# Dhia-naouali/dinov3-jax

Hardware: NVIDIA H100
Metric: global_crops_per_sec (higher is better)
Workload: dtype bf16

## Files before the change

dinov3-jax_b200/csrc/gemm_tc.cu:

```cuda
#include <cstdlib>
#include <cstring>
#include "ptx.cuh"
#include "d3_internal.h"

namespace d3 {

constexpr int BM = 128;
constexpr int BK = 64;
constexpr int GEMM_THREADS = 384;

constexpr int EPI_RUNTIME = -1;
constexpr int EPI_FLAGS = EP_BIAS | EP_GELU | EP_STORE_PRE | EP_MUL_DGELU | EP_GAMMA | EP_RESID | EP_OUT_F32 | EP_ACCUM |
                          EP_SLABS | EP_GELU_ERF;

template <int EF>
constexpr bool kStaged = EF != EPI_RUNTIME && (EF & (EP_SLABS | EP_ACCUM)) == 0;

template <int EF>
__device__ __forceinline__ bool epi_has(const GemmEpilogue& ep, int f) {
  return EF == EPI_RUNTIME ? (ep.flags & f) != 0 : (EF & f) != 0;
}

__device__ __forceinline__ float gelu_grad_epi(float u) {
  const float u2 = __fmul_rn(u, u);
  const float t = tanh_approx(__fmul_rn(u, fmaf(0.0356774081363001f, u2, 0.7978845608028654f)));
  const float dz = fmaf(0.1070322244089003f, u2, 0.7978845608028654f);
  return fmaf(__fmul_rn(__fmul_rn(0.5f, u), fmaf(-t, t, 1.0f)), dz, __fmul_rn(0.5f, __fadd_rn(1.0f, t)));
}

__device__ __forceinline__ float gelu_erf_epi(float u) {
  return __fmul_rn(__fmul_rn(0.5f, u), __fadd_rn(1.0f, erff(__fmul_rn(u, 0.70710678118654752f))));
}

template <int EF>
__device__ __forceinline__ float epi_value(const GemmEpilogue& ep, float acc, float bias, float u, float gamma,
                                           float resid, float old, float& pre) {
  float v = __fmul_rn(acc, ep.alpha);
  if (epi_has<EF>(ep, EP_BIAS)) v = __fadd_rn(v, bias);
  pre = v;
  if (epi_has<EF>(ep, EP_GELU)) v = gelu_tanh_fast(v);
  if (epi_has<EF>(ep, EP_GELU_ERF)) v = gelu_erf_epi(v);
  if (epi_has<EF>(ep, EP_MUL_DGELU)) v = __fmul_rn(v, gelu_grad_epi(u));
  if (epi_has<EF>(ep, EP_GAMMA)) v = __fmul_rn(v, gamma);
  if (epi_has<EF>(ep, EP_RESID)) v = __fadd_rn(v, resid);
  if (epi_has<EF>(ep, EP_ACCUM)) v = __fadd_rn(v, old);
  return v;
}

__device__ __forceinline__ float2 ld_pair(const float* p, bool vec, bool two) {
  if (vec) return *reinterpret_cast<const float2*>(p);
  return make_float2(p[0], two ? p[1] : 0.f);
}
__device__ __forceinline__ float2 ld_pair(const __nv_bfloat16* p, bool vec, bool two) {
  if (vec) return unpack_bf16(*reinterpret_cast<const uint32_t*>(p));
  return make_float2(__bfloat162float(p[0]), two ? __bfloat162float(p[1]) : 0.f);
}
__device__ __forceinline__ void st_pair(float* p, float a, float b, bool vec, bool two) {
  if (vec) {
    *reinterpret_cast<float2*>(p) = make_float2(a, b);
  } else {
    p[0] = a;
    if (two) p[1] = b;
  }
}
__device__ __forceinline__ void st_pair(__nv_bfloat16* p, float a, float b, bool vec, bool two) {
  if (vec) {
    *reinterpret_cast<uint32_t*>(p) = pack_bf16(a, b);
  } else {
    p[0] = __float2bfloat16(a);
    if (two) p[1] = __float2bfloat16(b);
  }
}

template <int BN>
__device__ __forceinline__ void epilogue_tile_runtime(const GemmEpilogue& ep, float (&acc)[2][BN / 2], int m0, int n0,
                                                      int M, int N, size_t slab_row0, int r_in, int c_in) {
  float* const out_f = reinterpret_cast<float*>(ep.out);
  __nv_bfloat16* const out_h = reinterpret_cast<__nv_bfloat16*>(ep.out);
  const bool aligned = (ep.flags & EP_SLOW) == 0;
#pragma unroll
  for (int mh = 0; mh < 2; ++mh)
#pragma unroll
    for (int h = 0; h < 2; ++h) {
      const size_t row = (size_t)(m0 + mh * 64 + r_in + 8 * h);
      if (row >= (size_t)M) continue;
      const size_t orow = slab_row0 + row;
#pragma unroll
      for (int i = 0; i < BN / 8; ++i) {
        const int n = n0 + 8 * i + c_in;
        if (n >= N) break;
        const bool two = n + 1 < N, vec = aligned && two;
        float2 b{}, u{}, g{}, x{}, o{};
        if (epi_has<EPI_RUNTIME>(ep, EP_BIAS)) b = ld_pair(ep.bias + n, vec, two);
        if (epi_has<EPI_RUNTIME>(ep, EP_MUL_DGELU)) u = ld_pair(ep.aux_in + row * ep.ld_aux + n, vec, two);
        if (epi_has<EPI_RUNTIME>(ep, EP_GAMMA)) g = ld_pair(ep.gamma + n, vec, two);
        if (epi_has<EPI_RUNTIME>(ep, EP_RESID)) x = ld_pair(ep.resid + row * ep.ld_resid + n, vec, two);
        if (epi_has<EPI_RUNTIME>(ep, EP_ACCUM)) o = ld_pair(out_f + orow * ep.ld_out + n, vec, two);
        float p0, p1;
        const float v0 = epi_value<EPI_RUNTIME>(ep, acc[mh][4 * i + 2 * h], b.x, u.x, g.x, x.x, o.x, p0);
        const float v1 = epi_value<EPI_RUNTIME>(ep, acc[mh][4 * i + 2 * h + 1], b.y, u.y, g.y, x.y, o.y, p1);
        if (epi_has<EPI_RUNTIME>(ep, EP_SCATTER)) {
          const unsigned long long g_idx = (unsigned long long)ep.sc_off + orow * ep.ld_out + n;
          const unsigned long long shard = (unsigned long long)ep.sc_shard;
          const unsigned r = (unsigned)(g_idx / shard);
          float* const dst = ep.sc_peer[r] + (g_idx - r * shard);
          if (!two) atomicAdd(dst, v0);
          else atomicAdd(reinterpret_cast<float2*>(dst), make_float2(v0, v1));
          continue;
        }
        if (epi_has<EPI_RUNTIME>(ep, EP_STORE_PRE)) st_pair(ep.aux_out + row * ep.ld_aux + n, p0, p1, vec, two);
        if (epi_has<EPI_RUNTIME>(ep, EP_OUT_F32)) st_pair(out_f + orow * ep.ld_out + n, v0, v1, vec, two);
        else st_pair(out_h + orow * ep.ld_out + n, v0, v1, vec, two);
      }
    }
}

constexpr int STG_BOX = 64 * 128;
constexpr int STG_BYTES = 3 * STG_BOX;
__device__ __forceinline__ uint32_t sw128(int r, int byte) {
  return r * 128 + ((((byte >> 4) ^ r) & 7) << 4) + (byte & 15);
}

template <int MH, int BN, int EF>
__device__ __forceinline__ void epilogue_tile(const GemmEpilogue& ep, const CUtensorMap* tm_out,
                                              const CUtensorMap* tm_pre, float (&acc)[MH][BN / 2], const float* s_bias,
                                              const float* s_gamma, uint8_t* stg, int& seq, int bar, int t, int m0,
                                              int n0, int M, int N, size_t slab_row0, int r_in, int c_in) {
  constexpr bool STAGED = kStaged<EF>;
  constexpr bool F32 = (EF & EP_OUT_F32) != 0;
  constexpr int OUT_BOXES = F32 ? 2 : 1;
  constexpr int CHUNK = (OUT_BOXES + ((EF & EP_STORE_PRE) ? 1 : 0)) * STG_BOX;
  constexpr int NBUF = STG_BYTES / CHUNK;
  static_assert(NBUF >= 1, "a chunk must fit the staging area");
  float* const out_f = reinterpret_cast<float*>(ep.out);
  __nv_bfloat16* const out_h = reinterpret_cast<__nv_bfloat16*>(ep.out);
#pragma unroll
  for (int mh = 0; mh < MH; ++mh)
#pragma unroll
    for (int cb = 0; cb < BN / 64; ++cb) {
      const int row0 = m0 + mh * 64, col0 = n0 + cb * 64;
      if (row0 >= M || col0 >= N) continue;
      float2 xr[2][8], xo[2][8];
      uint32_t xu[2][8];
#pragma unroll
      for (int h = 0; h < 2; ++h) {
        const size_t row = (size_t)row0 + r_in + 8 * h;
#pragma unroll
        for (int i = 0; i < 8; ++i) {
          const int n = col0 + 8 * i + c_in;
          if (row < (size_t)M && n < N) {
            if (epi_has<EF>(ep, EP_RESID))
              xr[h][i] = *reinterpret_cast<const float2*>(ep.resid + row * ep.ld_resid + n);
            if (epi_has<EF>(ep, EP_MUL_DGELU))
              xu[h][i] = *reinterpret_cast<const uint32_t*>(ep.aux_in + row * ep.ld_aux + n);
            if (epi_has<EF>(ep, EP_ACCUM))
              xo[h][i] = *reinterpret_cast<const float2*>(out_f + (slab_row0 + row) * ep.ld_out + n);
          }
        }
      }
      uint8_t* const buf = stg + (seq % NBUF) * CHUNK;
      if constexpr (STAGED) {
        if (t == 0) tma_store_wait_read<NBUF - 1>();
        named_bar_sync(bar, 128);
      }
#pragma unroll
      for (int h = 0; h < 2; ++h) {
        const int r = r_in + 8 * h;
        const size_t row = (size_t)row0 + r;
#pragma unroll
        for (int i = 0; i < 8; ++i) {
          const int cl = cb * 64 + 8 * i + c_in;
          const int n = n0 + cl;
          const float2 b = epi_has<EF>(ep, EP_BIAS) ? *reinterpret_cast<const float2*>(s_bias + cl) : float2{};
          const float2 g = epi_has<EF>(ep, EP_GAMMA) ? *reinterpret_cast<const float2*>(s_gamma + cl) : float2{};
          const float2 u = epi_has<EF>(ep, EP_MUL_DGELU) ? unpack_bf16(xu[h][i]) : float2{};
          float p0, p1;
          const float v0 = epi_value<EF>(ep, acc[mh][4 * (cl >> 3) + 2 * h], b.x, u.x, g.x, xr[h][i].x, xo[h][i].x, p0);
          const float v1 = epi_value<EF>(ep, acc[mh][4 * (cl >> 3) + 2 * h + 1], b.y, u.y, g.y, xr[h][i].y, xo[h][i].y,
                                         p1);
          if constexpr (STAGED) {
            if (epi_has<EF>(ep, EP_STORE_PRE))
              *reinterpret_cast<uint32_t*>(buf + OUT_BOXES * STG_BOX + sw128(r, 16 * i + 2 * c_in)) = pack_bf16(p0, p1);
            if constexpr (F32) {
              *reinterpret_cast<float2*>(buf + (i >> 2) * STG_BOX + sw128(r, 32 * (i & 3) + 4 * c_in)) =
                  make_float2(v0, v1);
            } else {
              *reinterpret_cast<uint32_t*>(buf + sw128(r, 16 * i + 2 * c_in)) = pack_bf16(v0, v1);
            }
          } else if (row < (size_t)M && n < N) {
            if (epi_has<EF>(ep, EP_STORE_PRE)) st_pair(ep.aux_out + row * ep.ld_aux + n, p0, p1, true, true);
            if constexpr (F32) st_pair(out_f + (slab_row0 + row) * ep.ld_out + n, v0, v1, true, true);
            else st_pair(out_h + (slab_row0 + row) * ep.ld_out + n, v0, v1, true, true);
          }
        }
      }
      if constexpr (STAGED) {
        fence_proxy_async_smem();
        named_bar_sync(bar, 128);
        if (t == 0) {
          tma_store_2d(tm_out, buf, col0, row0);
          if (F32 && col0 + 32 < N) tma_store_2d(tm_out, buf + STG_BOX, col0 + 32, row0);
          if constexpr ((EF & EP_STORE_PRE) != 0) tma_store_2d(tm_pre, buf + OUT_BOXES * STG_BOX, col0, row0);
          tma_store_commit();
        }
        ++seq;
      }
    }
}

template <int BN, bool STAGED>
struct Cfg {
  static constexpr bool WIDE = BN == 256;
  static constexpr int STAGES = (BN == 256 ? 4 : BN == 128 ? 6 : 8) - (STAGED ? 1 : 0);
  static constexpr int A_BYTES = BM * BK * 2;
  static constexpr int B_BYTES = BN * BK * 2;
  static constexpr int STAGE_BYTES = A_BYTES + B_BYTES;
  static constexpr int BAR_BYTES = 256;
  static constexpr int VEC_BYTES = (WIDE ? 1 : 2) * 2 * BN * 4;
  static constexpr int VEC_END = STAGES * STAGE_BYTES + BAR_BYTES + VEC_BYTES;
  static constexpr int STG_OFF = (VEC_END + 1023) / 1024 * 1024;
  static constexpr int SMEM_BYTES = (STAGED ? STG_OFF + 2 * STG_BYTES : VEC_END) + 1024;
  static_assert(SMEM_BYTES <= 227 * 1024, "over the opt-in shared-memory limit");
};

struct WorkRange { int m0, n0, kb0, kb1, sp; };
template <int BN>
__device__ __forceinline__ WorkRange work_item(int w, int rank, int num_n, int num_tiles, int num_k, int splits) {
  const int tile = w % num_tiles, sp = w / num_tiles;
  const int per = (num_k + splits - 1) / splits;
  WorkRange r;
  if constexpr (BN == 256) {
    r.n0 = (tile % num_n) * BN;
    r.m0 = (2 * (tile / num_n) + rank) * BM;
  } else {
    r.n0 = (2 * (tile % num_n) + rank) * BN;
    r.m0 = (tile / num_n) * BM;
  }
  r.kb0 = sp * per;
  r.kb1 = min(num_k, r.kb0 + per);
  r.sp = sp;
  return r;
}

template <int MH, int BN, int A_MN, int B_MN>
__device__ __forceinline__ void mma_kblock(float (&acc)[MH][BN / 2], uint32_t sa, uint32_t sb, bool first) {
  const uint64_t bd = B_MN ? gmma_desc_sw128(sb, 8192, 1024) : gmma_desc_sw128(sb, 16, 1024);
  constexpr uint64_t a_adv = A_MN ? (2048 >> 4) : (32 >> 4);
  constexpr uint64_t b_adv = B_MN ? (2048 >> 4) : (32 >> 4);
#pragma unroll
  for (int k = 0; k < BK / 16; ++k) {
    const uint32_t sc = (first && k == 0) ? 0u : 1u;
#pragma unroll
    for (int mh = 0; mh < MH; ++mh) {
      const uint64_t ad = A_MN ? gmma_desc_sw128(sa + mh * 8192, 8192, 1024) : gmma_desc_sw128(sa + mh * 8192, 16, 1024);
      if constexpr (BN == 256) wgmma_m64n256k16_ss<A_MN, B_MN>(acc[mh], ad + k * a_adv, bd + k * b_adv, sc);
      else if constexpr (BN == 128) wgmma_m64n128k16_ss<A_MN, B_MN>(acc[mh], ad + k * a_adv, bd + k * b_adv, sc);
      else wgmma_m64n64k16_ss<A_MN, B_MN>(acc[mh], ad + k * a_adv, bd + k * b_adv, sc);
    }
  }
}

template <int MH, int BN>
__device__ __forceinline__ void mma_khalf_e4m3(float (&acc)[MH][BN / 2], uint32_t sa, uint32_t sb, int h) {
  static_assert(BN == 64, "the e4m3 GEMM runs 128 x 64 tiles");
  const uint64_t bd = gmma_desc_sw128(sb, 16, 1024);
#pragma unroll
  for (int k = 0; k < 2; ++k) {
#pragma unroll
    for (int mh = 0; mh < MH; ++mh) {
      const uint64_t ad = gmma_desc_sw128(sa + mh * 8192, 16, 1024);
      wgmma_m64n64k32_e4m3(acc[mh], ad + (2 * h + k) * (32 >> 4), bd + (2 * h + k) * (32 >> 4), k == 0 ? 0u : 1u);
    }
  }
}

template <int MH, int BN>
__device__ __forceinline__ void add_acc(float (&acc)[MH][BN / 2], const float (&part)[MH][BN / 2]) {
#pragma unroll
  for (int mh = 0; mh < MH; ++mh)
#pragma unroll
    for (int i = 0; i < BN / 2; ++i) acc[mh][i] = __fadd_rn(acc[mh][i], part[mh][i]);
}

template <int BN, int A_MN, int B_MN, int EF, bool E4M3 = false>
__global__ void __launch_bounds__(GEMM_THREADS, 1)
gemm_kernel(const __grid_constant__ CUtensorMap tmA, const __grid_constant__ CUtensorMap tmB,
            const __grid_constant__ CUtensorMap tmO, const __grid_constant__ CUtensorMap tmP, const GemmEpilogue ep,
            int M, int N, int K, int splits, const float* scale_a, const float* scale_b) {
  static_assert(!E4M3 || (BN == 64 && !A_MN && !B_MN), "e4m3: 128 x 64 tiles, both operands K-major");
  constexpr int KB = E4M3 ? 128 : BK;
  constexpr bool staged = kStaged<EF>;
  using C = Cfg<BN, staged>;
  constexpr bool WIDE = C::WIDE;
  constexpr int MH = WIDE ? 1 : 2;
  static_assert(!WIDE || EF != EPI_RUNTIME, "run-time flags run on the 128-wide tile");
  static_assert(2 * C::STAGES * 8 <= C::BAR_BYTES, "mbarriers overflow their slot");
  extern __shared__ uint8_t smem_raw[];
  uint8_t* smem = reinterpret_cast<uint8_t*>((reinterpret_cast<uintptr_t>(smem_raw) + 1023) & ~uintptr_t(1023));
  uint64_t* full_bar = reinterpret_cast<uint64_t*>(smem + C::STAGES * C::STAGE_BYTES);
  uint64_t* empty_bar = full_bar + C::STAGES;
  float* vecs = reinterpret_cast<float*>(smem + C::STAGES * C::STAGE_BYTES + C::BAR_BYTES);

  const int wg = threadIdx.x >> 7;
  const int rank = blockIdx.x & 1;
  const int cluster = blockIdx.x >> 1, num_clusters = gridDim.x >> 1;
  if (threadIdx.x == 0) {
    tma_prefetch_desc(&tmA);
    tma_prefetch_desc(&tmB);
    if constexpr (staged) {
      tma_prefetch_desc(&tmO);
      if constexpr ((EF & EP_STORE_PRE) != 0) tma_prefetch_desc(&tmP);
    }
    for (int s = 0; s < C::STAGES; ++s) { mbar_init(&full_bar[s], 1); mbar_init(&empty_bar[s], WIDE ? 4 : 2); }
    fence_mbar_init();
  }
  cluster_sync();

  const int num_m = (M + BM - 1) / BM;
  const int num_n = WIDE ? (N + BN - 1) / BN : ((N + BN - 1) / BN + 1) / 2;
  const int num_k = (K + KB - 1) / KB;
  const int num_tiles = (WIDE ? (num_m + 1) / 2 : num_m) * num_n;
  const int num_work = num_tiles * splits;

  if (wg == 0) {
    setmaxnreg_dec<40>();
    if (threadIdx.x < 32 && elect_one()) {
      int stage = 0;
      uint32_t phase = 0;
      for (int w = cluster; w < num_work; w += num_clusters) {
        const WorkRange wr = work_item<BN>(w, rank, num_n, num_tiles, num_k, splits);
        for (int kb = wr.kb0; kb < wr.kb1; ++kb) {
          mbar_wait(&empty_bar[stage], phase ^ 1);
          uint8_t* sa = smem + stage * C::STAGE_BYTES;
          uint8_t* sb = sa + C::A_BYTES;
          mbar_expect_tx(&full_bar[stage], C::STAGE_BYTES);
          if constexpr (WIDE) {
#pragma unroll
            for (int i = 0; i < 2; ++i) {
              if (A_MN) tma_load_2d(&tmA, &full_bar[stage], sa + i * 8192, wr.m0 + i * 64, kb * KB);
              else tma_load_2d(&tmA, &full_bar[stage], sa + i * 8192, kb * KB, wr.m0 + i * 64);
            }
            if (B_MN) {
#pragma unroll
              for (int i = 2 * rank; i < 2 * rank + 2; ++i)
                tma_load_2d_multicast(&tmB, &full_bar[stage], sb + i * 8192, wr.n0 + i * 64, kb * KB, 0b11);
            } else {
              tma_load_2d_multicast(&tmB, &full_bar[stage], sb + rank * 16384, kb * KB, wr.n0 + rank * 128, 0b11);
            }
          } else {
            if (A_MN) {
              tma_load_2d_multicast(&tmA, &full_bar[stage], sa + rank * 8192, wr.m0 + rank * 64, kb * KB, 0b11);
            } else {
              tma_load_2d_multicast(&tmA, &full_bar[stage], sa + rank * 8192, kb * KB, wr.m0 + rank * 64, 0b11);
            }
            if (B_MN) {
#pragma unroll
              for (int i = 0; i < BN / 64; ++i) tma_load_2d(&tmB, &full_bar[stage], sb + i * 8192, wr.n0 + i * 64, kb * KB);
            } else {
              tma_load_2d(&tmB, &full_bar[stage], sb, kb * KB, wr.n0);
            }
          }
          if (++stage == C::STAGES) { stage = 0; phase ^= 1; }
        }
      }
    }
  } else {
    setmaxnreg_inc<232>();
    const int cw = wg - 1;
    const int t = threadIdx.x & 127;
    const int r_in = 16 * (t >> 5) + ((t & 31) >> 2);
    const int c_in = 2 * (t & 3);
    float* const s_bias = vecs + (WIDE ? 0 : cw * 2 * BN);
    float* const s_gamma = s_bias + BN;
    constexpr bool stage_vecs = EF != EPI_RUNTIME && (EF & (EP_BIAS | EP_GAMMA)) != 0;
    constexpr int VEC_THREADS = WIDE ? 256 : 128;
    const int vt = WIDE ? threadIdx.x - 128 : t;
    uint8_t* const stg = smem + C::STG_OFF + cw * STG_BYTES;
    const uint32_t peer_empty = mapa_shared(smem_u32(empty_bar), rank ^ 1);
    int stg_seq = 0;
    int stage = 0;
    uint32_t phase = 0;
    int j = 0;
    for (int w = cluster; w < num_work; w += num_clusters, ++j) {
      const WorkRange wr = work_item<BN>(w, rank, num_n, num_tiles, num_k, splits);
      const int nkb = wr.kb1 > wr.kb0 ? wr.kb1 - wr.kb0 : 0;
      if (!WIDE && (j & 1) != cw) {
        stage += nkb;
        phase ^= (stage / C::STAGES) & 1;
        stage %= C::STAGES;
        continue;
      }
      if constexpr (stage_vecs) {
        named_bar_sync(3 + cw * !WIDE, VEC_THREADS);
        if (vt < BN && wr.n0 + vt < N) {
          if constexpr ((EF & EP_BIAS) != 0) cp_async_4(s_bias + vt, ep.bias + wr.n0 + vt);
          if constexpr ((EF & EP_GAMMA) != 0) cp_async_4(s_gamma + vt, ep.gamma + wr.n0 + vt);
        }
      }
      if (!WIDE && j > 0) named_bar_sync(1 + cw, 256);
      float acc[MH][BN / 2];
#pragma unroll
      for (int mh = 0; mh < MH; ++mh)
#pragma unroll
        for (int i = 0; i < BN / 2; ++i) acc[mh][i] = 0.f;
      if constexpr (E4M3) {
        float part[MH][BN / 2];
        for (int kb = wr.kb0; kb < wr.kb1; ++kb) {
          mbar_wait(&full_bar[stage], phase);
          const uint32_t sa = smem_u32(smem + stage * C::STAGE_BYTES);
#pragma unroll
          for (int h = 0; h < 2; ++h) {
#pragma unroll
            for (int mh = 0; mh < MH; ++mh) fence_regs(part[mh]);
            wgmma_fence();
            mma_khalf_e4m3<MH, BN>(part, sa, sa + C::A_BYTES, h);
            wgmma_commit();
            wgmma_wait<0>();
#pragma unroll
            for (int mh = 0; mh < MH; ++mh) fence_regs(part[mh]);
            if (h == 1 && t == 0) { mbar_arrive(&empty_bar[stage]); mbar_arrive_cluster(peer_empty + 8 * stage); }
            add_acc<MH, BN>(acc, part);
          }
          if (++stage == C::STAGES) { stage = 0; phase ^= 1; }
        }
        if (!WIDE && w + num_clusters < num_work) named_bar_arrive(1 + (cw ^ 1), 256);
#pragma unroll
        for (int mh = 0; mh < MH; ++mh)
#pragma unroll
          for (int h = 0; h < 2; ++h) {
            const int row = wr.m0 + mh * 64 + r_in + 8 * h;
            const float s_row = row < M ? scale_a[row] : 0.f;
#pragma unroll
            for (int i = 0; i < BN / 8; ++i) {
              const int n = wr.n0 + 8 * i + c_in;
              const float s0 = n < N ? scale_b[n] : 0.f, s1 = n + 1 < N ? scale_b[n + 1] : 0.f;
              acc[mh][4 * i + 2 * h] = __fmul_rn(__fmul_rn(acc[mh][4 * i + 2 * h], s_row), s0);
              acc[mh][4 * i + 2 * h + 1] = __fmul_rn(__fmul_rn(acc[mh][4 * i + 2 * h + 1], s_row), s1);
            }
          }
      } else {
        int prev = -1;
        for (int kb = wr.kb0; kb < wr.kb1; ++kb) {
          mbar_wait(&full_bar[stage], phase);
          const uint32_t sa = smem_u32(smem + stage * C::STAGE_BYTES);
#pragma unroll
          for (int mh = 0; mh < MH; ++mh) fence_regs(acc[mh]);
          wgmma_fence();
          mma_kblock<MH, BN, A_MN, B_MN>(acc, sa + (WIDE ? cw * 8192 : 0), sa + C::A_BYTES, kb == wr.kb0);
          wgmma_commit();
#pragma unroll
          for (int mh = 0; mh < MH; ++mh) fence_regs(acc[mh]);
          if (prev >= 0) {
            wgmma_wait<1>();
            if (t == 0) { mbar_arrive(&empty_bar[prev]); mbar_arrive_cluster(peer_empty + 8 * prev); }
          }
          prev = stage;
          if (++stage == C::STAGES) { stage = 0; phase ^= 1; }
        }
        if (!WIDE && w + num_clusters < num_work) named_bar_arrive(1 + (cw ^ 1), 256);
        wgmma_wait<0>();
#pragma unroll
        for (int mh = 0; mh < MH; ++mh) fence_regs(acc[mh]);
        if (prev >= 0 && t == 0) { mbar_arrive(&empty_bar[prev]); mbar_arrive_cluster(peer_empty + 8 * prev); }
      }
      if constexpr (stage_vecs) {
        cp_async_wait_all();
        named_bar_sync(3 + cw * !WIDE, VEC_THREADS);
      }
      if (nkb <= 0) continue;
      const size_t slab_row0 = epi_has<EF>(ep, EP_SLABS) ? (size_t)wr.sp * M : 0;
      if constexpr (EF == EPI_RUNTIME) {
        epilogue_tile_runtime<BN>(ep, acc, wr.m0, wr.n0, M, N, slab_row0, r_in, c_in);
      } else {
        epilogue_tile<MH, BN, EF>(ep, &tmO, &tmP, acc, s_bias, s_gamma, stg, stg_seq, 5 + cw, t,
                                  wr.m0 + (WIDE ? cw * 64 : 0), wr.n0, M, N, slab_row0, r_in, c_in);
      }
    }
    if (staged && t == 0) tma_store_wait_all();
  }
  cluster_sync();
}

static int make_operand_map(CUtensorMap* map, const void* ptr, int mn, int k, int ld, int is_mn_major, int box_mn) {
  cuuint64_t dims[2], strides[1];
  cuuint32_t box[2], estr[2] = {1, 1};
  if (is_mn_major) {
    dims[0] = (cuuint64_t)mn; dims[1] = (cuuint64_t)k; box[0] = 64; box[1] = 64;
  } else {
    dims[0] = (cuuint64_t)k; dims[1] = (cuuint64_t)mn; box[0] = 64; box[1] = (cuuint32_t)box_mn;
  }
  strides[0] = (cuuint64_t)ld * 2;
  return encode_tensor_map_2d_bf16(map, ptr, dims, strides, box, estr);
}

template <int BN, int A_MN, int B_MN, int EF, bool E4M3 = false>
static int launch(const CUtensorMap& ta, const CUtensorMap& tb, const GemmEpilogue& ep, int M, int N, int K,
                  int splits, cudaStream_t stream, const float* scale_a = nullptr, const float* scale_b = nullptr) {
  using C = Cfg<BN, kStaged<EF>>;
  auto kern = gemm_kernel<BN, A_MN, B_MN, EF, E4M3>;
  cudaLaunchAttribute attr{};
  attr.id = cudaLaunchAttributeClusterDimension;
  attr.val.clusterDim.x = 2;
  attr.val.clusterDim.y = 1;
  attr.val.clusterDim.z = 1;
  cudaLaunchConfig_t cfg{};
  cfg.blockDim = dim3(GEMM_THREADS);
  cfg.dynamicSmemBytes = C::SMEM_BYTES;
  cfg.stream = stream;
  cfg.attrs = &attr;
  cfg.numAttrs = 1;
  static int max_clusters = 0;
  if (max_clusters == 0) {
    cudaError_t e = cudaFuncSetAttribute(kern, cudaFuncAttributeMaxDynamicSharedMemorySize, C::SMEM_BYTES);
    if (e != cudaSuccess) return set_error(D3_ERR_CUDA, cudaGetErrorString(e));
    cfg.gridDim = dim3(2 * sm_count());
    e = cudaOccupancyMaxActiveClusters(&max_clusters, kern, &cfg);
    if (e != cudaSuccess) return set_error(D3_ERR_CUDA, cudaGetErrorString(e));
    if (max_clusters < 1) return set_error(D3_ERR_CUDA, "gemm: no 2-CTA cluster fits on the device");
  }
  CUtensorMap to{}, tp{};
  if constexpr (kStaged<EF>) {
    const int elt = (EF & EP_OUT_F32) ? 4 : 2;
    int rc = encode_tensor_map_2d(&to, ep.out, elt, N, M, (cuuint64_t)ep.ld_out * elt, 128 / elt, 64, 128);
    if (rc) return rc;
    if constexpr ((EF & EP_STORE_PRE) != 0) {
      rc = encode_tensor_map_2d(&tp, ep.aux_out, 2, N, M, (cuuint64_t)ep.ld_aux * 2, 64, 64, 128);
      if (rc) return rc;
    }
  }
  const int num_m = (M + BM - 1) / BM, num_n = (N + BN - 1) / BN;
  const int work = (BN == 256 ? (num_m + 1) / 2 * num_n : num_m * ((num_n + 1) / 2)) * splits;
  cfg.gridDim = dim3(2 * (work < max_clusters ? work : max_clusters));
  cudaError_t e = cudaLaunchKernelEx(&cfg, kern, ta, tb, to, tp, ep, M, N, K, splits, scale_a, scale_b);
  if (e == cudaSuccess) e = cudaPeekAtLastError();
  if (e != cudaSuccess) return set_error(D3_ERR_CUDA, cudaGetErrorString(e));
  count_launch();
  return D3_OK;
}

template <int BN>
static int dispatch(int a_mn, int b_mn, const CUtensorMap& ta, const CUtensorMap& tb, const GemmEpilogue& ep, int M,
                    int N, int K, int splits, cudaStream_t s) {
  if (!(ep.flags & (EP_SLOW | EP_SCATTER)) && N % 2 == 0) {
    const int f = ep.flags & EPI_FLAGS;
#define D3_EPI(A, B, F) \
    if (a_mn == A && b_mn == B && f == (F)) return launch<BN, A, B, (F)>(ta, tb, ep, M, N, K, splits, s);
    D3_EPI(0, 1, 0)
    D3_EPI(0, 1, EP_BIAS)
    D3_EPI(0, 1, EP_BIAS | EP_OUT_F32)
    D3_EPI(0, 1, EP_BIAS | EP_GELU)
    D3_EPI(0, 1, EP_BIAS | EP_GELU | EP_STORE_PRE)
    D3_EPI(0, 1, EP_BIAS | EP_GAMMA | EP_RESID | EP_OUT_F32)
    D3_EPI(0, 1, EP_BIAS | EP_STORE_PRE | EP_GAMMA | EP_RESID | EP_OUT_F32)
    D3_EPI(0, 1, EP_BIAS | EP_GELU | EP_GAMMA | EP_RESID | EP_OUT_F32)
    D3_EPI(0, 1, EP_BIAS | EP_GELU | EP_STORE_PRE | EP_GAMMA | EP_RESID | EP_OUT_F32)
    D3_EPI(0, 1, EP_OUT_F32)
    D3_EPI(0, 1, EP_BIAS | EP_GELU_ERF)
    D3_EPI(0, 0, 0)
    D3_EPI(0, 0, EP_MUL_DGELU)
    D3_EPI(0, 0, EP_OUT_F32)
    D3_EPI(1, 1, EP_OUT_F32 | EP_SLABS)
    D3_EPI(1, 1, EP_OUT_F32 | EP_ACCUM)
#undef D3_EPI
  }
  if constexpr (BN == 256) {
    return dispatch<128>(a_mn, b_mn, ta, tb, ep, M, N, K, splits, s);
  } else {
    if (!a_mn && !b_mn) return launch<BN, 0, 0, EPI_RUNTIME>(ta, tb, ep, M, N, K, splits, s);
    if (!a_mn && b_mn) return launch<BN, 0, 1, EPI_RUNTIME>(ta, tb, ep, M, N, K, splits, s);
    if (a_mn && !b_mn) return launch<BN, 1, 0, EPI_RUNTIME>(ta, tb, ep, M, N, K, splits, s);
    return launch<BN, 1, 1, EPI_RUNTIME>(ta, tb, ep, M, N, K, splits, s);
  }
}

int gemm_bf16(const void* A, int lda, int a_mn, const void* B, int ldb, int b_mn, int M, int N, int K,
              GemmEpilogue ep, int tile_n, int split_k, cudaStream_t stream) {
  if (M <= 0 || N <= 0 || K <= 0) return set_error(D3_ERR_ARG, "gemm: empty problem");
  if ((lda % 8) || (ldb % 8) || (reinterpret_cast<uintptr_t>(A) & 15) || (reinterpret_cast<uintptr_t>(B) & 15))
    return set_error(D3_ERR_ARG, "gemm: operands must be 16-byte aligned with ld % 8 == 0");
  const int sms = sm_count();
  const int num_k = (K + BK - 1) / BK;
  int bn = tile_n >= 256 ? 256 : tile_n;
  if (tile_n == 0) {
    const int cand[2] = {128, 64};
    long best = -1;
    for (int i = 0; i < 2; ++i) {
      const long tiles = (long)((M + BM - 1) / BM) * ((N + cand[i] - 1) / cand[i]);
      const long waves = (tiles + sms - 1) / sms;
      const long cost = waves * (cand[i] + 24);
      if (best < 0 || cost < best) { best = cost; bn = cand[i]; }
    }
  }
  const bool plain_f32 = (ep.flags & EP_OUT_F32) && !(ep.flags & (EP_BIAS | EP_GELU | EP_STORE_PRE | EP_MUL_DGELU |
                                                                  EP_GAMMA | EP_RESID | EP_GELU_ERF));
  int splits = 1;
  if (split_k >= 1) {
    splits = split_k;
  } else if (plain_f32 && (ep.flags & EP_ACCUM)) {
    const int unit_n = bn < 128 ? bn : 128;
    const long units = (long)((M + BM - 1) / BM) * ((N + unit_n - 1) / unit_n);
    if (units <= sms && num_k >= 16) {
      splits = units * 2 <= sms ? (int)(sms / units) : 1;
      if (splits < (num_k + 63) / 64) splits = (num_k + 63) / 64;
      if (splits > num_k / 4) splits = num_k / 4;
      if (splits < 1) splits = 1;
    }
  }
  if (tile_n == 0 && a_mn && b_mn) bn = 256;
  if (ep.flags & EP_SCATTER) {
    if (!plain_f32) return set_error(D3_ERR_ARG, "gemm: SCATTER needs a plain fp32 output");
    if (ep.sc_world < 1 || ep.sc_world > 8 || ep.sc_shard <= 0 || (ep.sc_shard % 4) || (ep.sc_off % 4) || (ep.ld_out % 4))
      return set_error(D3_ERR_ARG, "gemm: SCATTER needs 1..8 ranks and 4-element aligned shard / offset / ld_out");
    if ((unsigned long long)ep.sc_off + (unsigned long long)(M - 1) * ep.ld_out + N > (unsigned long long)ep.sc_shard * ep.sc_world)
      return set_error(D3_ERR_ARG, "gemm: SCATTER output exceeds the sharded range");
  }
  if (splits > 1) {
    if (!plain_f32) return set_error(D3_ERR_ARG, "gemm: split-K needs a plain fp32 output");
    if (!(ep.flags & EP_ACCUM)) return set_error(D3_ERR_ARG, "gemm: split-K accumulates into out (set ACCUM, zero it first)");
    if (splits > num_k) splits = num_k;
  }
  if (ep.flags & EP_SCATTER) ep.flags &= ~EP_ACCUM;
  const int out_elt = (ep.flags & EP_OUT_F32) ? 4 : 2;
  bool aligned = ((uintptr_t)ep.out % 16 == 0) && ((ep.ld_out * out_elt) % 16 == 0);
  if (ep.flags & EP_BIAS) aligned = aligned && ((uintptr_t)ep.bias % 16 == 0);
  if (ep.flags & EP_GAMMA) aligned = aligned && ((uintptr_t)ep.gamma % 16 == 0);
  if (ep.flags & EP_RESID) aligned = aligned && ((uintptr_t)ep.resid % 16 == 0) && (ep.ld_resid % 4 == 0);
  if (ep.flags & EP_STORE_PRE) aligned = aligned && ((uintptr_t)ep.aux_out % 16 == 0) && (ep.ld_aux % 8 == 0);
  if (ep.flags & EP_MUL_DGELU) aligned = aligned && ((uintptr_t)ep.aux_in % 16 == 0) && (ep.ld_aux % 8 == 0);
  if (!aligned) ep.flags |= EP_SLOW;

  CUtensorMap ta, tb;
  int rc = make_operand_map(&ta, A, M, K, lda, a_mn, 64);
  if (rc) return rc;
  rc = make_operand_map(&tb, B, N, K, ldb, b_mn, bn < 128 ? bn : 128);
  if (rc) return rc;
  float* ws = nullptr;
  GemmEpilogue out_ep = ep;
  if (splits > 1 && !(ep.flags & EP_SCATTER)) {
    ws = slab_workspace((size_t)splits * M * N, stream);
    if (!ws) return D3_ERR_CUDA;
    ep.out = ws;
    ep.ld_out = N;
    ep.flags = (ep.flags & ~(EP_ACCUM | EP_SLOW)) | EP_SLABS | (N % 4 ? EP_SLOW : 0);
  }
  switch (bn) {
    case 256: rc = dispatch<256>(a_mn, b_mn, ta, tb, ep, M, N, K, splits, stream); break;
    case 128: rc = dispatch<128>(a_mn, b_mn, ta, tb, ep, M, N, K, splits, stream); break;
    case 64: rc = dispatch<64>(a_mn, b_mn, ta, tb, ep, M, N, K, splits, stream); break;
    default: rc = set_error(D3_ERR_ARG, "gemm: bad tile N");
  }
  if (ws) {
    if (!rc) rc = slab_combine(ws, splits, (long long)M * N, M, N, reinterpret_cast<float*>(out_ep.out), out_ep.ld_out, stream);
    slab_release(ws, stream);
  }
  return rc;
}

static int dispatch_e4m3(const CUtensorMap& ta, const CUtensorMap& tb, const GemmEpilogue& ep, int M, int N, int K,
                         const float* sa, const float* sb, cudaStream_t s) {
  if (!(ep.flags & EP_SLOW) && N % 2 == 0) {
    const int f = ep.flags & EPI_FLAGS;
#define D3_EPI(F) \
    if (f == (F)) return launch<64, 0, 0, (F), true>(ta, tb, ep, M, N, K, 1, s, sa, sb);
    D3_EPI(0)
    D3_EPI(EP_BIAS)
    D3_EPI(EP_BIAS | EP_GELU)
    D3_EPI(EP_BIAS | EP_GELU | EP_STORE_PRE)
    D3_EPI(EP_BIAS | EP_GAMMA | EP_RESID | EP_OUT_F32)
    D3_EPI(EP_BIAS | EP_STORE_PRE | EP_GAMMA | EP_RESID | EP_OUT_F32)
    D3_EPI(EP_BIAS | EP_GELU | EP_GAMMA | EP_RESID | EP_OUT_F32)
    D3_EPI(EP_BIAS | EP_GELU | EP_STORE_PRE | EP_GAMMA | EP_RESID | EP_OUT_F32)
    D3_EPI(EP_MUL_DGELU)
    D3_EPI(EP_OUT_F32)
    D3_EPI(EP_OUT_F32 | EP_ACCUM)
#undef D3_EPI
  }
  return launch<64, 0, 0, EPI_RUNTIME, true>(ta, tb, ep, M, N, K, 1, s, sa, sb);
}

int gemm_e4m3(const void* A, int lda, const float* sa, const void* B, int ldb, const float* sb, int M, int N, int K,
              GemmEpilogue ep, cudaStream_t stream) {
  if (M <= 0 || N <= 0 || K <= 0) return set_error(D3_ERR_ARG, "gemm_e4m3: empty problem");
  if (K % 16) return set_error(D3_ERR_ARG, "gemm_e4m3: K must be a multiple of 16");
  if ((lda % 16) || (ldb % 16) || (reinterpret_cast<uintptr_t>(A) & 15) || (reinterpret_cast<uintptr_t>(B) & 15))
    return set_error(D3_ERR_ARG, "gemm_e4m3: operands must be 16-byte aligned with ld % 16 == 0");
  if (ep.flags & (EP_SCATTER | EP_GELU_ERF)) return set_error(D3_ERR_ARG, "gemm_e4m3: SCATTER / GELU_ERF not supported");
  const int out_elt = (ep.flags & EP_OUT_F32) ? 4 : 2;
  bool aligned = ((uintptr_t)ep.out % 16 == 0) && ((ep.ld_out * out_elt) % 16 == 0);
  if (ep.flags & EP_BIAS) aligned = aligned && ((uintptr_t)ep.bias % 16 == 0);
  if (ep.flags & EP_GAMMA) aligned = aligned && ((uintptr_t)ep.gamma % 16 == 0);
  if (ep.flags & EP_RESID) aligned = aligned && ((uintptr_t)ep.resid % 16 == 0) && (ep.ld_resid % 4 == 0);
  if (ep.flags & EP_STORE_PRE) aligned = aligned && ((uintptr_t)ep.aux_out % 16 == 0) && (ep.ld_aux % 8 == 0);
  if (ep.flags & EP_MUL_DGELU) aligned = aligned && ((uintptr_t)ep.aux_in % 16 == 0) && (ep.ld_aux % 8 == 0);
  if (!aligned) ep.flags |= EP_SLOW;
  CUtensorMap ta, tb;
  int rc = encode_tensor_map_2d_u8(&ta, A, K, M, lda, 128, 64);
  if (rc) return rc;
  rc = encode_tensor_map_2d_u8(&tb, B, K, N, ldb, 128, 64);
  if (rc) return rc;
  return dispatch_e4m3(ta, tb, ep, M, N, K, sa, sb, stream);
}

}
```

Measured before the change: 540.7.

## Prefetch epilogue operands via TMA loader warps and software-pipelined residual loads

Reworks the staged GEMM epilogue's shared-memory staging into a per-box ring. Producer warps TMA-load the bf16 GELU-derivative input (aux_in) into ring slots ahead of the consumer, synchronised by new full/empty mbarriers. The residual tile for the next 64x64 chunk is prefetched in halves while the current chunk is computed. TMA stores are now committed per box so slots can be reused sooner. The aim is to hide global-load latency in the epilogue, at the cost of more mbarrier handshakes, extra registers and more complex synchronisation.

```diff
diff --git a/dinov3-jax_b200/csrc/gemm_tc.cu b/dinov3-jax_b200/csrc/gemm_tc.cu
--- a/dinov3-jax_b200/csrc/gemm_tc.cu
+++ b/dinov3-jax_b200/csrc/gemm_tc.cu
@@ -116,76 +116,102 @@
 }
 
 constexpr int STG_BOX = 64 * 128;
-constexpr int STG_BYTES = 3 * STG_BOX;
+constexpr int STG_SLOTS = 3;
+constexpr int STG_BYTES = STG_SLOTS * STG_BOX;
 __device__ __forceinline__ uint32_t sw128(int r, int byte) {
   return r * 128 + ((((byte >> 4) ^ r) & 7) << 4) + (byte & 15);
 }
+
+template <int EF>
+constexpr bool kLoader = kStaged<EF> && (EF & EP_MUL_DGELU) != 0;
 
 template <int MH, int BN, int EF>
 __device__ __forceinline__ void epilogue_tile(const GemmEpilogue& ep, const CUtensorMap* tm_out,
                                               const CUtensorMap* tm_pre, float (&acc)[MH][BN / 2], const float* s_bias,
-                                              const float* s_gamma, uint8_t* stg, int& seq, int bar, int t, int m0,
-                                              int n0, int M, int N, size_t slab_row0, int r_in, int c_in) {
+                                              const float* s_gamma, uint8_t* stg, uint64_t* slot_full,
+                                              uint64_t* slot_empty, int& seq, int bar, int t, int m0, int n0, int M,
+                                              int N, size_t slab_row0, int r_in, int c_in) {
   constexpr bool STAGED = kStaged<EF>;
+  constexpr bool LOAD = kLoader<EF>;
   constexpr bool F32 = (EF & EP_OUT_F32) != 0;
   constexpr int OUT_BOXES = F32 ? 2 : 1;
-  constexpr int CHUNK = (OUT_BOXES + ((EF & EP_STORE_PRE) ? 1 : 0)) * STG_BOX;
-  constexpr int NBUF = STG_BYTES / CHUNK;
-  static_assert(NBUF >= 1, "a chunk must fit the staging area");
+  constexpr int BOXES = OUT_BOXES + ((EF & EP_STORE_PRE) ? 1 : 0);
+  static_assert(BOXES <= STG_SLOTS, "a chunk must fit the staging ring");
+  static_assert(!LOAD || BOXES == 1, "the loader fills one box per chunk, STG_SLOTS chunks ahead");
+  constexpr bool PIPE = STAGED && (EF & EP_RESID) != 0;
+  constexpr int HALVES = PIPE ? 2 : 1, IW = 8 / HALVES;
+  constexpr int CB = BN / 64;
   float* const out_f = reinterpret_cast<float*>(ep.out);
   __nv_bfloat16* const out_h = reinterpret_cast<__nv_bfloat16*>(ep.out);
+  float2 xr[2][8];
+  auto load_resid = [&](int row0, int col0, int i0, int i1) {
+#pragma unroll
+    for (int h = 0; h < 2; ++h) {
+      const size_t row = (size_t)row0 + r_in + 8 * h;
+#pragma unroll
+      for (int i = i0; i < i1; ++i) {
+        const int n = col0 + 8 * i + c_in;
+        if (row < (size_t)M && n < N) xr[h][i] = *reinterpret_cast<const float2*>(ep.resid + row * ep.ld_resid + n);
+      }
+    }
+  };
 #pragma unroll
   for (int mh = 0; mh < MH; ++mh)
 #pragma unroll
-    for (int cb = 0; cb < BN / 64; ++cb) {
+    for (int cb = 0; cb < CB; ++cb) {
       const int row0 = m0 + mh * 64, col0 = n0 + cb * 64;
       if (row0 >= M || col0 >= N) continue;
-      float2 xr[2][8], xo[2][8];
-      uint32_t xu[2][8];
+      const int nrow0 = cb + 1 < CB ? row0 : row0 + 64, ncol0 = cb + 1 < CB ? col0 + 64 : n0;
+      const bool next = mh * CB + cb + 1 < MH * CB && nrow0 < M && ncol0 < N;
+      const bool preloaded = PIPE && (cb > 0 || (mh > 0 && n0 + (CB - 1) * 64 < N));
+      if (epi_has<EF>(ep, EP_RESID) && !preloaded) load_resid(row0, col0, 0, 8);
+      float2 xo[2][8];
 #pragma unroll
       for (int h = 0; h < 2; ++h) {
         const size_t row = (size_t)row0 + r_in + 8 * h;
 #pragma unroll
         for (int i = 0; i < 8; ++i) {
           const int n = col0 + 8 * i + c_in;
-          if (row < (size_t)M && n < N) {
-            if (epi_has<EF>(ep, EP_RESID))
-              xr[h][i] = *reinterpret_cast<const float2*>(ep.resid + row * ep.ld_resid + n);
-            if (epi_has<EF>(ep, EP_MUL_DGELU))
-              xu[h][i] = *reinterpret_cast<const uint32_t*>(ep.aux_in + row * ep.ld_aux + n);
-            if (epi_has<EF>(ep, EP_ACCUM))
-              xo[h][i] = *reinterpret_cast<const float2*>(out_f + (slab_row0 + row) * ep.ld_out + n);
-          }
+          if (epi_has<EF>(ep, EP_ACCUM) && row < (size_t)M && n < N)
+            xo[h][i] = *reinterpret_cast<const float2*>(out_f + (slab_row0 + row) * ep.ld_out + n);
         }
       }
-      uint8_t* const buf = stg + (seq % NBUF) * CHUNK;
-      if constexpr (STAGED) {
-        if (t == 0) tma_store_wait_read<NBUF - 1>();
+      uint8_t* const box0 = stg + (seq % STG_SLOTS) * STG_BOX;
+      uint8_t* const box1 = stg + ((seq + 1) % STG_SLOTS) * STG_BOX;
+      uint8_t* const box2 = stg + ((seq + 2) % STG_SLOTS) * STG_BOX;
+      uint8_t* const pre_box = OUT_BOXES == 1 ? box1 : box2;
+      if constexpr (LOAD) {
+        mbar_wait(&slot_full[seq % STG_SLOTS], (seq / STG_SLOTS) & 1);
+      } else if constexpr (STAGED) {
+        if (t == 0) tma_store_wait_read<STG_SLOTS - BOXES>();
         named_bar_sync(bar, 128);
       }
+#pragma unroll
+      for (int hf = 0; hf < HALVES; ++hf) {
 #pragma unroll
       for (int h = 0; h < 2; ++h) {
         const int r = r_in + 8 * h;
         const size_t row = (size_t)row0 + r;
 #pragma unroll
-        for (int i = 0; i < 8; ++i) {
+        for (int i = hf * IW; i < hf * IW + IW; ++i) {
           const int cl = cb * 64 + 8 * i + c_in;
           const int n = n0 + cl;
           const float2 b = epi_has<EF>(ep, EP_BIAS) ? *reinterpret_cast<const float2*>(s_bias + cl) : float2{};
           const float2 g = epi_has<EF>(ep, EP_GAMMA) ? *reinterpret_cast<const float2*>(s_gamma + cl) : float2{};
-          const float2 u = epi_has<EF>(ep, EP_MUL_DGELU) ? unpack_bf16(xu[h][i]) : float2{};
+          float2 u{};
+          if constexpr (LOAD) u = unpack_bf16(*reinterpret_cast<const uint32_t*>(box0 + sw128(r, 16 * i + 2 * c_in)));
           float p0, p1;
           const float v0 = epi_value<EF>(ep, acc[mh][4 * (cl >> 3) + 2 * h], b.x, u.x, g.x, xr[h][i].x, xo[h][i].x, p0);
           const float v1 = epi_value<EF>(ep, acc[mh][4 * (cl >> 3) + 2 * h + 1], b.y, u.y, g.y, xr[h][i].y, xo[h][i].y,
                                          p1);
           if constexpr (STAGED) {
             if (epi_has<EF>(ep, EP_STORE_PRE))
-              *reinterpret_cast<uint32_t*>(buf + OUT_BOXES * STG_BOX + sw128(r, 16 * i + 2 * c_in)) = pack_bf16(p0, p1);
+              *reinterpret_cast<uint32_t*>(pre_box + sw128(r, 16 * i + 2 * c_in)) = pack_bf16(p0, p1);
             if constexpr (F32) {
-              *reinterpret_cast<float2*>(buf + (i >> 2) * STG_BOX + sw128(r, 32 * (i & 3) + 4 * c_in)) =
+              *reinterpret_cast<float2*>((i >> 2 ? box1 : box0) + sw128(r, 32 * (i & 3) + 4 * c_in)) =
                   make_float2(v0, v1);
             } else {
-              *reinterpret_cast<uint32_t*>(buf + sw128(r, 16 * i + 2 * c_in)) = pack_bf16(v0, v1);
+              *reinterpret_cast<uint32_t*>(box0 + sw128(r, 16 * i + 2 * c_in)) = pack_bf16(v0, v1);
             }
           } else if (row < (size_t)M && n < N) {
             if (epi_has<EF>(ep, EP_STORE_PRE)) st_pair(ep.aux_out + row * ep.ld_aux + n, p0, p1, true, true);
@@ -194,16 +220,30 @@
           }
         }
       }
+      if constexpr (PIPE) {
+        if (next) load_resid(nrow0, ncol0, hf * IW, hf * IW + IW);
+      }
+      }
       if constexpr (STAGED) {
         fence_proxy_async_smem();
         named_bar_sync(bar, 128);
         if (t == 0) {
-          tma_store_2d(tm_out, buf, col0, row0);
-          if (F32 && col0 + 32 < N) tma_store_2d(tm_out, buf + STG_BOX, col0 + 32, row0);
-          if constexpr ((EF & EP_STORE_PRE) != 0) tma_store_2d(tm_pre, buf + OUT_BOXES * STG_BOX, col0, row0);
+          tma_store_2d(tm_out, box0, col0, row0);
           tma_store_commit();
+          if constexpr (F32) {
+            if (col0 + 32 < N) tma_store_2d(tm_out, box1, col0 + 32, row0);
+            tma_store_commit();
+          }
+          if constexpr ((EF & EP_STORE_PRE) != 0) {
+            tma_store_2d(tm_pre, pre_box, col0, row0);
+            tma_store_commit();
+          }
+          if constexpr (LOAD) {
+            tma_store_wait_read<1>();
+            if (seq > 0) mbar_arrive(&slot_empty[(seq - 1) % STG_SLOTS]);
+          }
         }
-        ++seq;
+        seq += BOXES;
       }
     }
 }
@@ -285,20 +325,24 @@
 template <int BN, int A_MN, int B_MN, int EF, bool E4M3 = false>
 __global__ void __launch_bounds__(GEMM_THREADS, 1)
 gemm_kernel(const __grid_constant__ CUtensorMap tmA, const __grid_constant__ CUtensorMap tmB,
-            const __grid_constant__ CUtensorMap tmO, const __grid_constant__ CUtensorMap tmP, const GemmEpilogue ep,
-            int M, int N, int K, int splits, const float* scale_a, const float* scale_b) {
+            const __grid_constant__ CUtensorMap tmO, const __grid_constant__ CUtensorMap tmP,
+            const __grid_constant__ CUtensorMap tmU, const GemmEpilogue ep, int M, int N, int K, int splits,
+            const float* scale_a, const float* scale_b) {
   static_assert(!E4M3 || (BN == 64 && !A_MN && !B_MN), "e4m3: 128 x 64 tiles, both operands K-major");
   constexpr int KB = E4M3 ? 128 : BK;
   constexpr bool staged = kStaged<EF>;
+  constexpr bool loader = kLoader<EF>;
   using C = Cfg<BN, staged>;
   constexpr bool WIDE = C::WIDE;
   constexpr int MH = WIDE ? 1 : 2;
   static_assert(!WIDE || EF != EPI_RUNTIME, "run-time flags run on the 128-wide tile");
-  static_assert(2 * C::STAGES * 8 <= C::BAR_BYTES, "mbarriers overflow their slot");
+  static_assert((2 * C::STAGES + 4 * STG_SLOTS) * 8 <= C::BAR_BYTES, "mbarriers overflow their slot");
   extern __shared__ uint8_t smem_raw[];
   uint8_t* smem = reinterpret_cast<uint8_t*>((reinterpret_cast<uintptr_t>(smem_raw) + 1023) & ~uintptr_t(1023));
   uint64_t* full_bar = reinterpret_cast<uint64_t*>(smem + C::STAGES * C::STAGE_BYTES);
   uint64_t* empty_bar = full_bar + C::STAGES;
+  uint64_t* slot_full = empty_bar + C::STAGES;
+  uint64_t* slot_empty = slot_full + 2 * STG_SLOTS;
   float* vecs = reinterpret_cast<float*>(smem + C::STAGES * C::STAGE_BYTES + C::BAR_BYTES);
 
   const int wg = threadIdx.x >> 7;
@@ -310,8 +354,11 @@
     if constexpr (staged) {
       tma_prefetch_desc(&tmO);
       if constexpr ((EF & EP_STORE_PRE) != 0) tma_prefetch_desc(&tmP);
+      if constexpr (loader) tma_prefetch_desc(&tmU);
     }
     for (int s = 0; s < C::STAGES; ++s) { mbar_init(&full_bar[s], 1); mbar_init(&empty_bar[s], WIDE ? 4 : 2); }
+    if constexpr (loader)
+      for (int s = 0; s < 2 * STG_SLOTS; ++s) { mbar_init(&slot_full[s], 1); mbar_init(&slot_empty[s], 1); }
     fence_mbar_init();
   }
   cluster_sync();
@@ -362,6 +409,26 @@
           }
           if (++stage == C::STAGES) { stage = 0; phase ^= 1; }
         }
+      }
+    } else if (loader && threadIdx.x >= 32 && threadIdx.x < 96 && elect_one()) {
+      const int cw = (threadIdx.x >> 5) - 1;
+      uint8_t* const stg = smem + C::STG_OFF + cw * STG_BYTES;
+      int q = 0, j = 0;
+      for (int w = cluster; w < num_work; w += num_clusters, ++j) {
+        if (!WIDE && (j & 1) != cw) continue;
+        const WorkRange wr = work_item<BN>(w, rank, num_n, num_tiles, num_k, splits);
+        if (wr.kb1 <= wr.kb0) continue;
+        const int m0 = wr.m0 + (WIDE ? cw * 64 : 0);
+        for (int mh = 0; mh < MH; ++mh)
+          for (int cb = 0; cb < BN / 64; ++cb) {
+            const int row0 = m0 + mh * 64, col0 = wr.n0 + cb * 64;
+            if (row0 >= M || col0 >= N) continue;
+            const int s = cw * STG_SLOTS + q % STG_SLOTS;
+            mbar_wait(&slot_empty[s], ((q / STG_SLOTS) & 1) ^ 1);
+            mbar_expect_tx(&slot_full[s], STG_BOX);
+            tma_load_2d_cta(&tmU, &slot_full[s], stg + (q % STG_SLOTS) * STG_BOX, col0, row0);
+            ++q;
+          }
       }
     }
   } else {
@@ -472,8 +539,9 @@
       if constexpr (EF == EPI_RUNTIME) {
         epilogue_tile_runtime<BN>(ep, acc, wr.m0, wr.n0, M, N, slab_row0, r_in, c_in);
       } else {
-        epilogue_tile<MH, BN, EF>(ep, &tmO, &tmP, acc, s_bias, s_gamma, stg, stg_seq, 5 + cw, t,
-                                  wr.m0 + (WIDE ? cw * 64 : 0), wr.n0, M, N, slab_row0, r_in, c_in);
+        epilogue_tile<MH, BN, EF>(ep, &tmO, &tmP, acc, s_bias, s_gamma, stg, slot_full + cw * STG_SLOTS,
+                                  slot_empty + cw * STG_SLOTS, stg_seq, 5 + cw, t, wr.m0 + (WIDE ? cw * 64 : 0), wr.n0,
+                                  M, N, slab_row0, r_in, c_in);
       }
     }
     if (staged && t == 0) tma_store_wait_all();
@@ -518,7 +586,7 @@
     if (e != cudaSuccess) return set_error(D3_ERR_CUDA, cudaGetErrorString(e));
     if (max_clusters < 1) return set_error(D3_ERR_CUDA, "gemm: no 2-CTA cluster fits on the device");
   }
-  CUtensorMap to{}, tp{};
+  CUtensorMap to{}, tp{}, tu{};
   if constexpr (kStaged<EF>) {
     const int elt = (EF & EP_OUT_F32) ? 4 : 2;
     int rc = encode_tensor_map_2d(&to, ep.out, elt, N, M, (cuuint64_t)ep.ld_out * elt, 128 / elt, 64, 128);
@@ -527,11 +595,15 @@
       rc = encode_tensor_map_2d(&tp, ep.aux_out, 2, N, M, (cuuint64_t)ep.ld_aux * 2, 64, 64, 128);
       if (rc) return rc;
     }
+    if constexpr (kLoader<EF>) {
+      rc = encode_tensor_map_2d(&tu, ep.aux_in, 2, N, M, (cuuint64_t)ep.ld_aux * 2, 64, 64, 128);
+      if (rc) return rc;
+    }
   }
   const int num_m = (M + BM - 1) / BM, num_n = (N + BN - 1) / BN;
   const int work = (BN == 256 ? (num_m + 1) / 2 * num_n : num_m * ((num_n + 1) / 2)) * splits;
   cfg.gridDim = dim3(2 * (work < max_clusters ? work : max_clusters));
-  cudaError_t e = cudaLaunchKernelEx(&cfg, kern, ta, tb, to, tp, ep, M, N, K, splits, scale_a, scale_b);
+  cudaError_t e = cudaLaunchKernelEx(&cfg, kern, ta, tb, to, tp, tu, ep, M, N, K, splits, scale_a, scale_b);
   if (e == cudaSuccess) e = cudaPeekAtLastError();
   if (e != cudaSuccess) return set_error(D3_ERR_CUDA, cudaGetErrorString(e));
   count_launch();
```

Result: no change. 543.9, median of 6 (+0.6%).
